# ZJULiHongxin/HRNet-Hand-Pose-Estimation

Measured on AMD Instinct MI355X. Metric: images/sec fwd+bwd pose_hrnet_w32 256x256 bs=64/GPU, higher is better.
Workload: dtype bf16; 1 GPU; pose_hrnet_w32 256x256 bf16 fwd+HeatmapLoss+bwd+Adam training step, batch 64/GPU, synthetic RHD-shaped crops, random-init weights; global_batch=64, parallelism=dp1

## Files before the change

### hrnet-hand-pose-estimation_amd/build.py

```python
import hashlib
import os
import subprocess
import sys
from concurrent.futures import ThreadPoolExecutor

HERE = os.path.dirname(os.path.abspath(__file__))
REPO = os.path.dirname(HERE)
CSRC = os.path.join(HERE, 'csrc')
OBJ = os.path.join(CSRC, 'build')
LIB = os.path.join(CSRC, 'libhrnet_hip.so')
SOURCES = ['api.hip', 'conv.hip', 'conv_bs.hip', 'conv_fwd.hip', 'conv_dg.hip', 'conv_fwdb.hip', 'conv_fwds.hip', 'conv_ring.hip', 'wgrad.hip', 'bwd_fused.hip', 'bwd_pw.hip', 'gemm_pw.hip', 'head_mix.hip', 'eltwise.hip', 'loss.hip', 'dcn.hip', 'preprocess.hip', 'triangulate.hip', 'volumetric.hip', 'conv3d.hip', 'conv3d_train.hip', 'pointwise.hip', 'view_fusion.hip', 'transformer.hip', 'swin.hip', 'nmf.hip']
HEADERS = [os.path.join(CSRC, 'common.h'), os.path.join(CSRC, 'conv_body.h'), os.path.join(CSRC, 'conv_ring.h'), os.path.join(REPO, 'include', 'hrnet_hip.h')]
HIPCC = os.environ.get('HIPCC', '/opt/rocm/bin/hipcc')
FLAGS = ['--offload-arch=gfx950', '-O3', '-std=c++17', '-fPIC', '-fno-gpu-rdc',
         '-I', os.path.join(REPO, 'include'), '-I', CSRC, '-Wno-unused-result']


EXTRA = {}


def _stamp(src):
    h = hashlib.sha1()
    for p in [src] + HEADERS:
        with open(p, 'rb') as f:
            h.update(f.read())
    h.update(' '.join(FLAGS + EXTRA.get(os.path.basename(src), [])).encode())
    return h.hexdigest()


def _compile(name):
    src = os.path.join(CSRC, name)
    obj = os.path.join(OBJ, name.replace('.hip', '.o'))
    stamp_file = obj + '.stamp'
    stamp = _stamp(src)
# ... 31 lines not shown
```

### hrnet-hand-pose-estimation_amd/csrc/common.h

```cpp
#pragma once
#include <stdlib.h>
#include <hip/hip_runtime.h>
#include <stdint.h>

#include "hrnet_hip.h"

typedef __bf16 bf16_t;
typedef float f32x4 __attribute__((ext_vector_type(4)));
typedef float f32x2 __attribute__((ext_vector_type(2)));
typedef __bf16 bf16x8 __attribute__((ext_vector_type(8)));
typedef __bf16 bf16x4 __attribute__((ext_vector_type(4)));
typedef uint32_t u32x4 __attribute__((ext_vector_type(4)));
typedef uint32_t u32x2 __attribute__((ext_vector_type(2)));
typedef u32x4 V16;

#define LDS_AS __attribute__((address_space(3)))

template <typename T>
struct TT;
template <>
struct TT<float> {
  static constexpr int VEC = 4;
  static constexpr int KSTEP = 16;
  static constexpr int ID = HR_F32;
// ... 234 lines not shown
int hr_launch_wgrad(const HrOp& op, hipStream_t s);
int hr_launch_wgrad_reduce(const HrOp& op, hipStream_t s);
int hr_launch_bn_finalize(const HrOp& op, hipStream_t s);
int hr_launch_sum_terms(const HrOp& op, hipStream_t s);
int hr_launch_grad_term(const HrOp& op, hipStream_t s);
int hr_launch_bn_bwd_reduce(const HrOp& op, hipStream_t s);
int hr_launch_bn_bwd_finalize(const HrOp& op, hipStream_t s);
int hr_launch_bilinear_cat(const HrOp& op, hipStream_t s);
int hr_launch_bilinear_cat_bwd(const HrOp& op, hipStream_t s);
int hr_launch_im2col_stem(const HrOp& op, hipStream_t s);
int hr_launch_nhwc_to_nchw(const HrOp& op, hipStream_t s);
int hr_launch_nchw_to_nhwc(const HrOp& op, hipStream_t s);
int hr_launch_pack_weights(const HrOp& op, hipStream_t s);
int hr_launch_bias_grad(const HrOp& op, hipStream_t s);
int hr_launch_fill(const HrOp& op, hipStream_t s);
int hr_launch_pack_table(const HrOp& op, hipStream_t s);
int hr_launch_wgrad_reduce_table(const HrOp& op, hipStream_t s);
int hr_launch_bwd_fused(const HrOp& op, hipStream_t s);
int hr_launch_bwd_pw(const HrOp& op, hipStream_t s);
int hr_launch_conv_sum(const HrOp& op, hipStream_t s);
int hr_gemm_pw_supported(int dtype, int Cin, int Cout);
int hr_gemm_pw(const void* x, const void* w, const float* bias, void* y, float* sums, long long pixels, int Cin,
               int Cout, hipStream_t s);
int hr_launch_bn_finalize_table(const HrOp& op, hipStream_t s);
int hr_launch_ew_table(const HrOp& op, hipStream_t s);
int hr_launch_head_mix(const HrOp& op, hipStream_t s);
int hr_launch_upsample_t(const HrOp& op, hipStream_t s);
int hr_launch_head_bwd(const HrOp& op, hipStream_t s);
int hr_launch_pool_reduce(const HrOp& op, hipStream_t s);
```

### hrnet-hand-pose-estimation_amd/csrc/conv.hip

```cpp
#include <string.h>

#include "conv_body.h"
#include "conv_ring.h"

HR_DEFINE_CONV_LAUNCH(hr_conv_launch_generic, CONV_GENERIC)

namespace {
inline int conv_xcd_runs() {
  static const int v = hr_knob("HRNET_CONV_XCD", 1);
  return v;
}
inline int conv_mode(const ConvArgs& a, bool in_relu) {
  if (a.bs_y) return CONV_BS;
  if (!a.bias && !a.upz && !a.accumulate && a.stats) return CONV_FWD;
  if (a.bias && !a.upz && !a.accumulate) return CONV_FWDB;
  if (!a.bias && !a.in_scale && !a.in_sums && !in_relu && !a.stats) return CONV_DG;
  return CONV_GENERIC;
}

inline int ring_serves(const ConvArgs& a, int dtype, int ks, int stride, int mode, bool in_relu) {
  if (ks != 3 || stride != 1 || a.upz || a.bias || a.in_dy || a.in_dx || !hr_conv_ring_enabled()) return 0;
  const bool raw = !a.in_scale && !a.in_sums && !in_relu;
  if (mode == CONV_BS || (raw && a.accumulate && !a.stats))
    return hr_conv_ring_supported(dtype, a.N, a.H, a.W, a.Cin, a.Cout, 1) ? 2 : 0;
// ... 83 lines not shown
             "conv2d: input batch sums need gamma/beta, no scale/shift arrays, Cin <= %d", HR_CONV_MAXC);
  HR_REQUIRE(!a.in_sums || !a.bs_y, "conv2d: batch-sum input is for forward launches");
  HR_REQUIRE(!a.bs_y || a.stats, "conv2d: backward statistics need a rows buffer");
  HR_REQUIRE(!a.bs_store_masked || a.bs_y, "conv2d: the masked store belongs to a backward-statistics launch");
  HR_REQUIRE(!a.bs_y || (!a.in_scale && !a.bias && !op.i[HR_CONV_I_IN_RELU]),
             "conv2d: backward statistics are for input-gradient launches (no input affine / ReLU / bias)");
  HR_REQUIRE((a.bs_scale == nullptr) == (a.bs_shift == nullptr), "conv2d: mask scale/shift must come together");
  a.N = N; a.H = H; a.W = W; a.Cin = Cin;
  a.Ho = Ho; a.Wo = Wo; a.Cout = Cout;
  a.in_relu = op.i[HR_CONV_I_IN_RELU]; a.upz = upz; a.accumulate = op.i[HR_CONV_I_ACCUMULATE];
  const int mode = conv_mode(a, op.i[HR_CONV_I_IN_RELU] != 0);
  HR_REQUIRE(!a.in_sums || mode == CONV_FWD || mode == CONV_FWDB,
             "conv2d: batch-sum input needs a forward launch that writes statistics or adds a bias");
  const int route = op.i[HR_CONV_I_ROUTE];
  HR_REQUIRE(route >= 0 && route <= 2, "conv2d: bad route %d", route);
  const int rs = route == 1 ? 0 : ring_serves(a, dtype, ks, op.i[HR_CONV_I_STRIDE], mode, op.i[HR_CONV_I_IN_RELU] != 0);
  HR_REQUIRE(route != 2 || rs, "conv2d: the op was recorded for the LDS-ring kernel, which does not serve it now "
             "(hrnet_conv_ring_enable() changed after the plan was recorded: record the plan again)");
  if (rs) return launch_ring(a, op.i[HR_CONV_I_IN_RELU], s);
  if (ks == 1 && stride == 1 && !upz && !a.accumulate && !a.bs_y && !a.in_scale && !a.in_sums &&
      !op.i[HR_CONV_I_IN_RELU] &&
      (!a.stats || a.stats_atomic) && !a.in_dy && !a.in_dx && hr_gemm_pw_supported(dtype, Cin, Cout))
    return hr_gemm_pw(a.x, a.w, a.bias, a.y, a.stats, (long long)N * H * W, Cin, Cout, s);
  const bool s2d = upz && (mode == CONV_BS || mode == CONV_DG);
  if (upz) {
    HR_REQUIRE(ks == 3, "conv2d: upz needs a 3x3 kernel");
    HR_REQUIRE((Ho + 1) / 2 == H && (Wo + 1) / 2 == W, "conv2d: upz shape mismatch");
    stride = s2d ? 4 : 1;
    if (s2d) { a.upz = 0; a.Hz = H; a.Wz = W; }
    else { a.Hz = Ho; a.Wz = Wo; }
  } else {
    const int pad = ks / 2;
    HR_REQUIRE((H + 2 * pad - ks) / stride + 1 == Ho && (W + 2 * pad - ks) / stride + 1 == Wo,
               "conv2d: output %dx%d does not match input %dx%d ks=%d stride=%d", Ho, Wo, H, W, ks, stride);
    a.Hz = H; a.Wz = W;
  }
  const TileChoice tc = choose_tile(N, Ho, Wo, Cout, ks, op.i[HR_CONV_I_STRIDE], op.p[HR_CONV_P_BS_Y] != nullptr, s2d);
  a.tiles_y = (Ho + tc.th - 1) / tc.th;
  a.tiles_x = (Wo + tc.tw - 1) / tc.tw;
  a.total_tiles = N * a.tiles_y * a.tiles_x;
  a.tpw = tc.tpw;
  a.gx = tc.gx;
  a.gy = (Cout + tc.bn - 1) / tc.bn;
  a.xcd_runs = conv_xcd_runs();
  ConvLaunch l;
  l.a = a; l.tc = tc; l.dtype = dtype; l.N = N; l.ks = ks; l.stride = stride;
// ... 140 lines not shown
  op.p[HR_CONV_P_X] = (void*)x; op.p[HR_CONV_P_WGT] = (void*)w; op.p[HR_CONV_P_Y] = y; op.p[HR_CONV_P_STATS] = stats;
  op.p[HR_CONV_P_BS_Y] = (void*)bs_y; op.p[HR_CONV_P_BS_MASK] = (void*)bs_mask;
  op.p[HR_CONV_P_BS_SCALE] = (void*)bs_scale; op.p[HR_CONV_P_BS_SHIFT] = (void*)bs_shift;
  HR_REQUIRE(bs_y, "conv2d_bwdstats: null bs_y");
  return hr_launch_conv(op, (hipStream_t)stream);
}

extern "C" int hrnet_conv_mode(int bwdstats, int has_bias, int upz, int accumulate, int has_stats, int has_affine,
                               int in_relu) {
  ConvArgs a = {};
  a.bs_y = bwdstats ? (const char*)1 : nullptr;
  a.bias = has_bias ? (const float*)1 : nullptr;
  a.upz = upz; a.accumulate = accumulate;
  a.stats = has_stats ? (float*)1 : nullptr;
  a.in_scale = has_affine ? (const float*)1 : nullptr;
  return conv_mode(a, in_relu != 0);
}

extern "C" int hrnet_conv_kernel_name(int dtype, int N, int Ho, int Wo, int Cin, int Cout, int ks, int stride,
                                      int upz, int mode, char* buf, int buflen) {
  if (ks == 1 && stride == 1 && !upz && hr_gemm_pw_supported(dtype, Cin, Cout) &&
      (mode == CONV_FWD || mode == CONV_FWDB || mode == CONV_DG))
    return snprintf(buf, buflen, "gemm_pw_kernel");
  if (ks == 3 && stride == 1 && !upz && mode == CONV_FWDS && hr_conv_ring_sum_supported(dtype, N, Ho, Wo, Cin, Cout)) {
    char tmp[96];
    hr_conv_ring_name(hr_conv_ring_supported(dtype, N, Ho, Wo, Cin, Cout, 0), 0, tmp, sizeof(tmp));
    const int n = (int)strlen(tmp);
    if (n > 1) tmp[n - 1] = 0;
    return snprintf(buf, buflen, "%s, true>", tmp);
  }
  if (ks == 3 && stride == 1 && !upz && hr_conv_ring_enabled()) {
    const int bsm = mode == CONV_BS ? 1 : 0;
    if ((bsm || mode == CONV_FWD || mode == CONV_GENERIC || mode == CONV_DG) &&
        hr_conv_ring_supported(dtype, N, Ho, Wo, Cin, Cout, bsm))
      return hr_conv_ring_name(hr_conv_ring_supported(dtype, N, Ho, Wo, Cin, Cout, bsm), bsm, buf, buflen);
  }
  const bool s2d = upz && (mode == CONV_BS || mode == CONV_DG);
  const TileChoice tc = choose_tile(N, Ho, Wo, Cout, ks, stride, mode == CONV_BS, s2d);
  static const int wp[8] = {4, 2, 2, 2, 2, 0, 4, 2}, wc[8] = {1, 2, 2, 2, 2, 0, 1, 2};
  const int kstride = s2d ? 4 : (ks == 1 || upz) ? 1 : stride;
  const int km = conv_km(dtype, ks, Cin, tc.id);
  static const char* names[6] = {"conv_kernel", "conv_bs_kernel", "conv_fwd_kernel", "conv_dg_kernel", "conv_fwdb_kernel",
                                 "conv_fwds_kernel"};
  return snprintf(buf, buflen, "%s<%s, %d, %d, %d, %d, %d, %d, %d, %d>", names[mode >= 0 && mode < 6 ? mode : 0],
                  dtype == HR_F32 ? "float" : "__bf16", ks, kstride, tc.th, tc.tw, tc.bn, wp[tc.id], wc[tc.id], km);
}
// ... 1 lines not shown
```

### hrnet-hand-pose-estimation_amd/csrc/eltwise.hip

```cpp
#include "common.h"

namespace {

constexpr int EW_BLOCK = 256;
inline unsigned ew_grid(long long n) {
  long long g = (n + EW_BLOCK - 1) / EW_BLOCK;
  if (g > 256LL * 16) g = 256LL * 16;
  if (g < 1) g = 1;
  return (unsigned)g;
}

constexpr int FIN_LANES = 32;
__device__ __forceinline__ void partial_sums(const float* rows, int n, int C, int c, int tl, int cl,
                                             double (*red)[FIN_LANES][32], double& s1, double& s2) {
  double a0 = 0, a1 = 0, b0 = 0, b1 = 0;
  if (c < C) {
    int t = tl;
    for (; t + FIN_LANES < n; t += 2 * FIN_LANES) {
      const float x0 = rows[((size_t)t * 2 + 0) * C + c], y0 = rows[((size_t)t * 2 + 1) * C + c];
      const float x1 = rows[((size_t)(t + FIN_LANES) * 2 + 0) * C + c];
      const float y1 = rows[((size_t)(t + FIN_LANES) * 2 + 1) * C + c];
      a0 += (double)x0; b0 += (double)y0; a1 += (double)x1; b1 += (double)y1;
    }
    if (t < n) {
// ... 918 lines not shown
      const int k = (int)(idx % Cin_pad);
      const int co = (int)(idx / Cin_pad);
      if (co < Cout && k < taps * Cin) {
        const int t = k / Cin, ci = k % Cin;
        val = w[((size_t)co * Cin + ci) * taps + t];
      }
    }
    out[idx] = (T)val;
  }
}

constexpr int PACK_LDS_FLOATS = 4864;
__host__ __device__ inline int pack_nci(int Cout, int taps) {
  for (int p = 16; p > 1; p >>= 1)
    if (Cout * (p * taps + 1) <= PACK_LDS_FLOATS) return p;
  return 1;
}
__host__ __device__ inline int pack_rows(int Cin_pad, int taps) {
  const int r = 2048 / (Cin_pad * taps);
  return r < 1 ? 1 : (r > 8 ? 8 : r);
}

template <typename T>
__global__ __launch_bounds__(256) void pack_table_kernel(const HrPackEnt* tab, int n) {
  __shared__ float buf[PACK_LDS_FLOATS];
  int lo = 0, hi = n - 1;
  while (lo < hi) {
    const int mid = (lo + hi + 1) >> 1;
    if (tab[mid].block0 <= (int)blockIdx.x) lo = mid; else hi = mid - 1;
  }
  const HrPackEnt e = tab[lo];
  const int taps = e.ks * e.ks;
  const float* w = (const float*)e.w;
  T* out = (T*)e.out;
  const int u = (int)blockIdx.x - e.block0;
  if (e.mode == 0) {
    const int nr = pack_rows(e.Cin_pad, taps), co0 = u * nr, rowlen = e.Cin * taps, olen = taps * e.Cin_pad;
    const int rows = e.Cout_pad - co0 < nr ? e.Cout_pad - co0 : nr;
    for (int i = threadIdx.x; i < rows * rowlen; i += 256) {
      const int r = i / rowlen;
      buf[i] = co0 + r < e.Cout ? w[e.ld ? (size_t)(co0 + r) * e.ld + (i - r * rowlen) : (size_t)co0 * rowlen + i] : 0.f;
    }
    __syncthreads();
    T* o = out + (size_t)co0 * olen;
    for (int idx = threadIdx.x; idx < rows * olen; idx += 256) {
      const int r = idx / olen, q = idx - r * olen;
      const int t = q / e.Cin_pad, ci = q - t * e.Cin_pad;
      o[idx] = (T)((co0 + r < e.Cout && ci < e.Cin) ? buf[r * rowlen + ci * taps + t] : 0.f);
    }
  } else if (e.mode == 1) {
    const int per = pack_nci(e.Cout_pad, taps);
    const int ci0 = u * per, span = per * taps, pitch = span + 1;
    const int nci = e.Cin_pad - ci0 < per ? e.Cin_pad - ci0 : per;
    for (int i = threadIdx.x; i < e.Cout * span; i += 256) {
      const int co = i / span, r = i - co * span;
      const int ci = ci0 + r / taps;
      buf[co * pitch + r] = ci < e.Cin ? w[((size_t)co * e.Cin + ci0) * taps + r] : 0.f;
    }
    __syncthreads();
    for (int idx = threadIdx.x; idx < nci * taps * e.Cout_pad; idx += 256) {
      const int co = idx % e.Cout_pad;
      const int tf = (idx / e.Cout_pad) % taps;
      const int cl = idx / (e.Cout_pad * taps);
      out[((size_t)(ci0 + cl) * taps + tf) * e.Cout_pad + co] =
          (T)(co < e.Cout ? buf[co * pitch + cl * taps + (taps - 1 - tf)] : 0.f);
    }
  } else {
    const long long total = (long long)e.Cout_pad * e.Cin_pad;
    const long long base = (long long)u * 1024;
#pragma unroll
    for (int r = 0; r < 4; ++r) {
      const long long idx = base + r * 256 + threadIdx.x;
      if (idx >= total) break;
      const int k = (int)(idx % e.Cin_pad);
      const int co = (int)(idx / e.Cin_pad);
      float val = 0.f;
      if (co < e.Cout && k < taps * e.Cin) val = w[((size_t)co * e.Cin + (k % e.Cin)) * taps + k / e.Cin];
      out[idx] = (T)val;
    }
  }
}

template <typename T>
__global__ __launch_bounds__(256) void colsum_kernel(const char* dy, float* partial, long long pixels,
                                                     int Cp) {
  constexpr int VEC = TT<T>::VEC;
  __shared__ float red[256 * VEC];
  const int cv = Cp / VEC;
  const int rows = 256 / cv;
  const int v = threadIdx.x % cv, row = threadIdx.x / cv;
  float s1[VEC];
#pragma unroll
  for (int j = 0; j < VEC; ++j) s1[j] = 0.f;
  if (row < rows)
    for (long long p = (long long)blockIdx.x * rows + row; p < pixels; p += (long long)gridDim.x * rows) {
      float f[VEC];
      v16_unpack<T>(*(const V16*)(dy + ((size_t)p * Cp + v * VEC) * sizeof(T)), f);
#pragma unroll
      for (int j = 0; j < VEC; ++j) s1[j] += f[j];
    }
#pragma unroll
  for (int j = 0; j < VEC; ++j) red[threadIdx.x * VEC + j] = s1[j];
  __syncthreads();
// ... 264 lines not shown
    if (op.i[HR_GRAD_TERM_I_DTYPE] == HR_F32)
      hipLaunchKernelGGL(grad_term_rows_kernel<float>, dim3(ew_grid(tot2)), dim3(256), 0, s, a);
    else
      hipLaunchKernelGGL(grad_term_rows_kernel<bf16_t>, dim3(ew_grid(tot2)), dim3(256), 0, s, a);
    return hr_check_launch("grad_term");
  }
  if (op.i[HR_GRAD_TERM_I_DTYPE] == HR_F32)
    hipLaunchKernelGGL(grad_term_kernel<float>, dim3(ew_grid(total)), dim3(256), 0, s, a);
  else
    hipLaunchKernelGGL(grad_term_kernel<bf16_t>, dim3(ew_grid(total)), dim3(256), 0, s, a);
  return hr_check_launch("grad_term");
}

extern "C" int hrnet_pack_blocks(int Cout_pad, int Cin_pad, int ks, int mode) {
  if (mode == 0) {
    const int nr = pack_rows(Cin_pad, ks * ks);
    return (Cout_pad + nr - 1) / nr;
  }
  if (mode == 1) {
    const int per = pack_nci(Cout_pad, ks * ks);
    return (Cin_pad + per - 1) / per;
  }
  return (int)(((long long)Cout_pad * Cin_pad + 1023) / 1024);
}

extern "C" int hrnet_reduce_blocks(int N, int H, int W, int C) {
  const long long npix = (long long)N * H * W;
  long long b = npix / 64;
  if (b < 1) b = 1;
  if (b > 2048) b = 2048;
  (void)C;
  return (int)b;
}

int hr_launch_bn_bwd_reduce(const HrOp& op, hipStream_t s) {
  GradArgs a;
  if (int e = fill_grad_args(op, a, true)) return e;
  const int vec = op.i[HR_BN_BWD_REDUCE_I_DTYPE] == HR_F32 ? 4 : 8;
  HR_REQUIRE(a.C / vec <= 256, "bn_bwd_reduce: C=%d too wide", a.C);
  const int blocks = hrnet_reduce_blocks(a.N, a.H, a.W, a.C);
  if (op.i[HR_BN_BWD_REDUCE_I_DTYPE] == HR_F32)
    hipLaunchKernelGGL(bn_bwd_reduce_kernel<float>, dim3(blocks), dim3(256), 0, s, a);
  else
    hipLaunchKernelGGL(bn_bwd_reduce_kernel<bf16_t>, dim3(blocks), dim3(256), 0, s, a);
  return hr_check_launch("bn_bwd_reduce");
}
// ... 395 lines not shown
```

### hrnet-hand-pose-estimation_amd/lib/hipnet/net.py

```python
import torch
import torch.nn as nn

from . import _capi as C
from . import ops
from .engine import BNRec, ConvRec, Plan, Program


class HipNet(object):
    def __init__(self, module, stage_cfg, compute_dtype):
        self.module = module
        self.stage_cfg = stage_cfg
        self.compute_dtype = compute_dtype
        self.dtid = C.dtype_id(compute_dtype)
        C.lib()
        params = list(module.parameters())
        if not params or not params[0].is_cuda:
            raise RuntimeError('pose_hrnet: parameters must live on a HIP device (model.cuda()); '
                               'there is no CPU path')
        self.device = params[0].device
        self.plans = {}
        self.fwd_packed = self.bwd_packed = False
        self._flatten(params)
        self._records()

# ... 50 lines not shown
        self.convs, self.bns, self.bn_list, self.bias_pad = {}, {}, {}, {}
        self.bn_list = []
        skip = tuple(getattr(self.module, 'hip_skip_prefixes', ()))
        for name, m in self.module.named_modules():
            if skip and name.startswith(skip):
                continue
            if isinstance(m, nn.Conv2d):
                r = ConvRec(name, m, stem=(name == 'conv1'))
                es = torch.empty((), dtype=self.compute_dtype).element_size()
                taps = r.ks * r.ks
                nf = r.Cout_pad * (1 if r.stem else taps) * r.Cin_pad
                r.wf = torch.empty(nf * es, dtype=torch.uint8, device=self.device)
                if not r.stem:
                    r.wd = torch.empty(r.Cin_pad * taps * r.Cout_pad * es, dtype=torch.uint8, device=self.device)
                self.convs[name] = r
                if m.bias is not None:
                    self.bias_pad[name] = torch.zeros(r.Cout_pad, dtype=torch.float32, device=self.device)
            elif isinstance(m, nn.BatchNorm2d):
                b = BNRec(name, m, self.device)
                self.bns[name] = b
                self.bn_list.append(b)
        self.pack_f = self._pack_program([(r, 2 if r.stem else 0, r.wf) for r in self.convs.values()])
        self.pack_d = self._pack_program([(r, 1, r.wd) for r in self.convs.values() if r.wd is not None])

    def _pack_program(self, items):
        import ctypes
        ents = (C.HrPackEnt * len(items))()
        block = 0
        for e, item in zip(ents, items):
            r, mode, out = item[:3]
            taps = r.ks * r.ks
            if (mode == 1 and r.Cout_pad * (taps + 1) > 4864) or (mode == 0 and r.Cin * taps > 4864):
                raise ValueError('{}: {} output channels at {}x{} exceed the LDS staging of the weight packer'.format(
                    r.prefix, r.Cout, r.ks, r.ks))
            e.w, e.out = C.ptr(r.mod.weight), C.ptr(out)
            e.Cout, e.Cin, e.ks, e.Cout_pad, e.Cin_pad, e.mode = r.Cout, r.Cin, r.ks, r.Cout_pad, r.Cin_pad, mode
            if len(item) > 3:
                c0, c = item[3], item[4]
                assert r.ks == 1 and mode == 0
                e.w = r.mod.weight.data_ptr() + 4 * c0
                e.Cin, e.Cin_pad, e.ld = c, c, r.Cin
            e.block0 = block
            block += C.call('hrnet_pack_blocks', e.Cout_pad, e.Cin_pad, r.ks, mode)
        raw = bytes(ctypes.string_at(ctypes.addressof(ents), ctypes.sizeof(ents)))
        table = torch.frombuffer(bytearray(raw), dtype=torch.uint8).to(self.device)
        self._tables = getattr(self, '_tables', []) + [table]
        prog = Program()
        prog.add(ops.make(C.OP_PACK_TABLE, dtype=self.dtid, n=len(items), blocks=block, table=C.ptr(table)))
        return prog.finalize()

    def head_slices(self, crec, widths):
        key = (crec.prefix, tuple(widths))
        if getattr(self, '_head_key', None) != key:
            es = torch.empty((), dtype=self.compute_dtype).element_size()
            items, off = [], 0
            self._head_wf = []
            for c in widths:
                out = torch.empty(crec.Cout_pad * c * es, dtype=torch.uint8, device=self.device)
                self._head_wf.append(out)
                items.append((crec, 0, out, off, c))
                off += c
            self._head_pack = self._pack_program(items)
            self._head_key = key
            self._head_pack.run()
        return self._head_wf

    def pack_weights(self, for_backward):
        if not self.fwd_packed:
            self.pack_f.run()
            if getattr(self, '_head_pack', None) is not None:
                self._head_pack.run()
            for name, buf in self.bias_pad.items():
                b = self.convs[name].mod.bias
                buf[:b.numel()].copy_(b.detach())
            self.fwd_packed = True
        if for_backward and not self.bwd_packed:
            self.pack_d.run()
            self.bwd_packed = True

    def mark_weights_dirty(self):
        self.fwd_packed = self.bwd_packed = False

    MAX_PLANS_IN_FLIGHT = 4

    def plan(self, N, H, W, training, need_grad):
        key = (N, H, W, bool(training), bool(need_grad))
        pool = self.plans.setdefault(key, [])
        for p in pool:
            if not (need_grad and p.busy):
                return p
        if len(pool) >= self.MAX_PLANS_IN_FLIGHT:
            raise RuntimeError('pose_hrnet: {} training forwards of shape {} are waiting for their backward; run '
                               'backward (or drop the outputs) before more forwards'.format(len(pool), (N, H, W)))
        p = Plan(self, N, H, W, training, need_grad)
        pool.append(p)
        return p

    def forward(self, x, training, need_grad):
        if x.dim() != 4 or x.shape[1] != 3:
            raise ValueError('pose_hrnet expects (B,3,H,W) input, got {}'.format(tuple(x.shape)))
# ... 38 lines not shown
```

### include/hrnet_hip.h

```cpp
#ifndef HRNET_HIP_H
#define HRNET_HIP_H

#include <stdint.h>

#ifdef __cplusplus
extern "C" {
#endif

#define HR_ABI_VERSION 2
#define HR_HOST

typedef void* hr_stream_t;
typedef int hr_value_t;

enum { HR_F32 = 0, HR_BF16 = 1 };

enum {
  HR_OK = 0,
  HR_E_BADARG = -1,
  HR_E_LAUNCH = -2,
  HR_E_BADOP = -3
};

enum {
// ... 161 lines not shown
void* hrnet_event_create(void);
int hrnet_event_destroy(void* event);

int hrnet_conv2d(int dtype, const void* x, const void* w, const float* in_scale,
                 const float* in_shift, const float* bias, void* y, float* stats, int N, int H,
                 int W, int Cin, int Ho, int Wo, int Cout, int ks, int stride, int upz,
                 int in_relu, int accumulate, hr_stream_t stream);

int hrnet_lincomb_f32(float* out, long long n, int k, HR_HOST const float* const* srcs, HR_HOST const float* coefs,
                      hr_stream_t stream);

int hrnet_conv2d_dilated3x3(int dtype, const void* x, const void* w_taps, long long tap_stride_bytes, void* y,
                            int N, int H, int W, int Cin, int Cout, int dilation, hr_stream_t stream);

int hrnet_conv2d_bwdstats(int dtype, const void* x, const void* w, void* y, float* stats,
                          const void* bs_y, const void* bs_mask, const float* bs_scale,
                          const float* bs_shift, int N, int H, int W, int Cin, int Ho, int Wo,
                          int Cout, int ks, int stride, int upz, int accumulate, hr_stream_t stream);
hr_value_t hrnet_conv_ring_enable(int on);
hr_value_t hrnet_conv_ring_supported(int dtype, int N, int H, int W, int Cin, int Cout);
hr_value_t hrnet_conv_rows_bwdstats(int dtype, int N, int Ho, int Wo, int Cin, int Cout, int ks, int stride);
hr_value_t hrnet_conv_route(int dtype, int N, int Ho, int Wo, int Cin, int Cout, int ks, int stride);
hr_value_t hrnet_conv_ring_sum_enable(int on);

hr_value_t hrnet_conv_kernel_name(int dtype, int N, int Ho, int Wo, int Cin, int Cout, int ks, int stride, int upz,
                                  int mode, HR_HOST char* buf, int buflen);
hr_value_t hrnet_conv_mode(int bwdstats, int has_bias, int upz, int accumulate, int has_stats, int has_affine,
                           int in_relu);
hr_value_t hrnet_wgrad_kernel_name(int dtype, int Ho, int Wo, int Cout, int Cin, int ks, int stride,
                                   HR_HOST char* buf, int buflen);
hr_value_t hrnet_conv_tiles(int N, int Ho, int Wo, int Cout, int ks, int stride);
hr_value_t hrnet_conv_tile_walk(int N, int Ho, int Wo, int Cout, int ks, int stride, int bwdstats, int s2d,
                                HR_HOST int* out5);
hr_value_t hrnet_conv_tiles_bwdstats(int N, int Ho, int Wo, int Cout, int ks, int stride);

int hrnet_conv2d_wgrad(int dtype, const void* x, const void* dy, const float* in_scale,
                       const float* in_shift, float* slabs, int N, int H, int W, int Cin, int Ho,
                       int Wo, int Cout, int ks, int stride, int in_relu, int nsplit,
                       hr_stream_t stream);
hr_value_t hrnet_wgrad_splits(int dtype, int N, int Ho, int Wo, int Cout, int Cin, int ks, int stride);
hr_value_t hrnet_wgrad_tiles(int dtype, int N, int Ho, int Wo, int Cout, int Cin, int ks, int stride);
hr_value_t hrnet_wgrad_blocks_per_split(int dtype, int Ho, int Wo, int Cout, int Cin, int ks, int stride);
int hrnet_wgrad_reduce(const float* slabs, float* grad_oihw, int nsplit, int Cout, int Cin,
                       int ks, int Cout_real, int Cin_real, int kflat, int accumulate,
                       hr_stream_t stream);

// ... 25 lines not shown
                            const void* addend, int mask_out, float* rows, const void* bs_y, float* slabs,
                            long long pixels, int Cin, int Cout, hr_stream_t stream);
int hrnet_conv1x1_bwd_fused_bnref(int dtype, const void* dz, const void* y, const float* coef, const HrBnBwdRef* ref,
                                  const void* x, const float* in_scale, const float* in_shift, int in_relu,
                                  const void* wT, void* dx, const void* addend, int mask_out, float* rows,
                                  const void* bs_y, float* slabs, long long pixels, int Cin, int Cout,
                                  hr_stream_t stream);
hr_value_t hrnet_bwd_pw_supported(int dtype, int Cin, int Cout);
hr_value_t hrnet_bwd_pw_rows_supported(int dtype, int Cin, int Cout);
hr_value_t hrnet_bwd_pw_splits(int dtype, long long pixels, int Cin, int Cout);
hr_value_t hrnet_bwd_pw_kernel_name(int dtype, int Cin, int Cout, HR_HOST char* buf, int buflen);

int hrnet_pack_weights(int dtype, const float* w_oihw, void* packed, int Cout, int Cin, int ks,
                       int Cout_pad, int Cin_pad, int mode, hr_stream_t stream);
typedef struct HrPackEnt {
  const void* w;
  void* out;
  int32_t Cout, Cin, ks, Cout_pad, Cin_pad, mode, block0;
  int32_t ld;
} HrPackEnt;
int hrnet_pack_weights_table(int dtype, const HrPackEnt* table, int n, int total_blocks,
                             hr_stream_t stream);
hr_value_t hrnet_pack_blocks(int Cout_pad, int Cin_pad, int ks, int mode);

typedef struct HrWredEnt {
  const float* slabs;
  float* grad;
  int32_t nsplit, Cout_pad, Cin_pad, ks, Cout, Cin, kflat, accumulate, block0;
  int32_t ld;
} HrWredEnt;
int hrnet_wgrad_reduce_table(const HrWredEnt* table, int n, int total_blocks, hr_stream_t stream);

int hrnet_bn_finalize(const float* stats, int tiles, int C, float count, const float* gamma,
                      const float* beta, float* running_mean, float* running_var,
                      int64_t* num_batches_tracked, float momentum, float eps, int training,
                      float* scale, float* shift, float* save_mean, float* save_invstd,
                      hr_stream_t stream);

int hrnet_conv2d_bnref(int dtype, const void* x, const void* w, const float* in_sums, const float* in_gamma,
                       const float* in_beta, float in_inv_count, float in_eps, const float* bias, void* y,
                       float* out_sums, int N, int H, int W, int Cin, int Ho, int Wo, int Cout, int ks, int stride,
                       int in_relu, hr_stream_t stream);
int hrnet_conv2d_sum(int dtype, const void* x, const void* x2, const void* w, const float* in_scale,
                     const float* in_shift, const float* in_sums, const float* in_gamma, const float* in_beta,
                     float in_inv_count, float in_eps, void* side, void* y, float* stats, int stats_atomic, int N,
                     int H, int W, int Cin, int Cout, int ks, hr_stream_t stream);
// ... 285 lines not shown
```

Measured before the change: 4342 images/sec.

## Add narrow pointwise conv kernel and fused forward/dgrad weight-pack pass

Adds a dedicated MFMA kernel for 1x1 bias convolutions with 16 or 32 output channels (e.g. the heatmap head). It keeps the weights in LDS, applies the input BN affine and ReLU on the fly, and prefetches activations several jobs deep. Separately, it adds a paired weight-pack kernel that reads each fp32 weight tile once into LDS and writes both the forward and the flipped dgrad packed layouts, plus the head slices, replacing two separate pack launches per step. These target a poorly served narrow GEMM and redundant weight reads, at the cost of more code paths to keep consistent.

After: 4385 images/sec (median of 6 runs). Within noise of the previous version (+1.0%).

```diff
diff --git a/hrnet-hand-pose-estimation_amd/build.py b/hrnet-hand-pose-estimation_amd/build.py
--- a/hrnet-hand-pose-estimation_amd/build.py
+++ b/hrnet-hand-pose-estimation_amd/build.py
@@ -9,7 +9,7 @@
 CSRC = os.path.join(HERE, 'csrc')
 OBJ = os.path.join(CSRC, 'build')
 LIB = os.path.join(CSRC, 'libhrnet_hip.so')
-SOURCES = ['api.hip', 'conv.hip', 'conv_bs.hip', 'conv_fwd.hip', 'conv_dg.hip', 'conv_fwdb.hip', 'conv_fwds.hip', 'conv_ring.hip', 'wgrad.hip', 'bwd_fused.hip', 'bwd_pw.hip', 'gemm_pw.hip', 'head_mix.hip', 'eltwise.hip', 'loss.hip', 'dcn.hip', 'preprocess.hip', 'triangulate.hip', 'volumetric.hip', 'conv3d.hip', 'conv3d_train.hip', 'pointwise.hip', 'view_fusion.hip', 'transformer.hip', 'swin.hip', 'nmf.hip']
+SOURCES = ['api.hip', 'conv.hip', 'conv_bs.hip', 'conv_fwd.hip', 'conv_dg.hip', 'conv_fwdb.hip', 'conv_fwds.hip', 'conv_ring.hip', 'wgrad.hip', 'bwd_fused.hip', 'bwd_pw.hip', 'gemm_pw.hip', 'conv_pwn.hip', 'head_mix.hip', 'eltwise.hip', 'loss.hip', 'dcn.hip', 'preprocess.hip', 'triangulate.hip', 'volumetric.hip', 'conv3d.hip', 'conv3d_train.hip', 'pointwise.hip', 'view_fusion.hip', 'transformer.hip', 'swin.hip', 'nmf.hip']
 HEADERS = [os.path.join(CSRC, 'common.h'), os.path.join(CSRC, 'conv_body.h'), os.path.join(CSRC, 'conv_ring.h'), os.path.join(REPO, 'include', 'hrnet_hip.h')]
 HIPCC = os.environ.get('HIPCC', '/opt/rocm/bin/hipcc')
 FLAGS = ['--offload-arch=gfx950', '-O3', '-std=c++17', '-fPIC', '-fno-gpu-rdc',
diff --git a/hrnet-hand-pose-estimation_amd/csrc/common.h b/hrnet-hand-pose-estimation_amd/csrc/common.h
--- a/hrnet-hand-pose-estimation_amd/csrc/common.h
+++ b/hrnet-hand-pose-estimation_amd/csrc/common.h
@@ -280,6 +280,12 @@
 int hr_gemm_pw_supported(int dtype, int Cin, int Cout);
 int hr_gemm_pw(const void* x, const void* w, const float* bias, void* y, float* sums, long long pixels, int Cin,
                int Cout, hipStream_t s);
+int hr_conv_pw_narrow_supported(int dtype, int Cin, int Cout);
+int hr_conv_pw_narrow_name(int Cout, char* buf, int buflen);
+int hr_conv_pw_narrow(const void* x, const void* w, const float* bias, void* y, const float* in_scale,
+                      const float* in_shift, const float* in_sums, const float* in_gamma, const float* in_beta,
+                      float in_inv_count, float in_eps, int in_relu, long long pixels, int Cin, int Cout,
+                      hipStream_t s);
 int hr_launch_bn_finalize_table(const HrOp& op, hipStream_t s);
 int hr_launch_ew_table(const HrOp& op, hipStream_t s);
 int hr_launch_head_mix(const HrOp& op, hipStream_t s);
diff --git a/hrnet-hand-pose-estimation_amd/csrc/conv.hip b/hrnet-hand-pose-estimation_amd/csrc/conv.hip
--- a/hrnet-hand-pose-estimation_amd/csrc/conv.hip
+++ b/hrnet-hand-pose-estimation_amd/csrc/conv.hip
@@ -129,6 +129,10 @@
       !op.i[HR_CONV_I_IN_RELU] &&
       (!a.stats || a.stats_atomic) && !a.in_dy && !a.in_dx && hr_gemm_pw_supported(dtype, Cin, Cout))
     return hr_gemm_pw(a.x, a.w, a.bias, a.y, a.stats, (long long)N * H * W, Cin, Cout, s);
+  if (mode == CONV_FWDB && ks == 1 && stride == 1 && Ho == H && Wo == W && !a.stats && !a.in_dy && !a.in_dx &&
+      hr_conv_pw_narrow_supported(dtype, Cin, Cout))
+    return hr_conv_pw_narrow(a.x, a.w, a.bias, a.y, a.in_scale, a.in_shift, a.in_sums, a.in_gamma, a.in_beta,
+                             a.in_inv_count, a.in_eps, a.in_relu, (long long)N * H * W, Cin, Cout, s);
   const bool s2d = upz && (mode == CONV_BS || mode == CONV_DG);
   if (upz) {
     HR_REQUIRE(ks == 3, "conv2d: upz needs a 3x3 kernel");
@@ -315,6 +319,8 @@
   if (ks == 1 && stride == 1 && !upz && hr_gemm_pw_supported(dtype, Cin, Cout) &&
       (mode == CONV_FWD || mode == CONV_FWDB || mode == CONV_DG))
     return snprintf(buf, buflen, "gemm_pw_kernel");
+  if (ks == 1 && stride == 1 && !upz && mode == CONV_FWDB && hr_conv_pw_narrow_supported(dtype, Cin, Cout))
+    return hr_conv_pw_narrow_name(Cout, buf, buflen);
   if (ks == 3 && stride == 1 && !upz && mode == CONV_FWDS && hr_conv_ring_sum_supported(dtype, N, Ho, Wo, Cin, Cout)) {
     char tmp[96];
     hr_conv_ring_name(hr_conv_ring_supported(dtype, N, Ho, Wo, Cin, Cout, 0), 0, tmp, sizeof(tmp));
diff --git a/hrnet-hand-pose-estimation_amd/csrc/conv_pwn.hip b/hrnet-hand-pose-estimation_amd/csrc/conv_pwn.hip
--- /dev/null
+++ b/hrnet-hand-pose-estimation_amd/csrc/conv_pwn.hip
@@ -0,0 +1,196 @@
+#include <stdio.h>
+
+#include "common.h"
+
+namespace {
+
+struct PwnArgs {
+  const char* x;
+  const char* w;
+  const float* bias;
+  char* y;
+  const float* in_scale;
+  const float* in_shift;
+  const float* in_sums;
+  const float* in_gamma;
+  const float* in_beta;
+  float in_inv_count, in_eps;
+  long long P;
+  int Cin, in_relu;
+};
+
+constexpr int PWN_MAXC = 768;
+constexpr int PWN_PF = 2;
+constexpr int PWN_D = 5;
+constexpr int PWN_JOB = 16 * PWN_PF;
+
+template <int FC>
+__global__ __launch_bounds__(256) void conv_pw_narrow_kernel(PwnArgs a) {
+  extern __shared__ __attribute__((aligned(16))) char lds[];
+  constexpr int LANE_C = 4 * FC;
+  const int tid = threadIdx.x, lane = tid & 63, wave = tid >> 6;
+  const int li = lane & 15, lg = lane >> 4;
+  const int Cin = a.Cin, nk = (Cin + 31) >> 5, kp = nk * 32, rowb = kp * 2 + 16;
+  char* wl = lds;
+  float* tab = (float*)(lds + 16 * FC * rowb);
+
+  const long long njobs = (a.P + PWN_JOB - 1) / PWN_JOB;
+  const long long gstride = (long long)gridDim.x * 4;
+  long long lj = (long long)blockIdx.x * 4 + wave, cj = lj;
+  int lk = 0, ck = 0;
+  V16 buf[PWN_D][PWN_PF];
+  auto issue = [&](V16* b) {
+#pragma unroll
+    for (int pf = 0; pf < PWN_PF; ++pf) {
+      long long p = lj * PWN_JOB + pf * 16 + li;
+      if (p >= a.P) p = a.P - 1;
+      const int c = min(lk * 32 + lg * 8, Cin - 8);
+      b[pf] = *(const V16*)(a.x + ((size_t)p * Cin + c) * 2);
+    }
+    if (++lk == nk) { lk = 0; lj += gstride; }
+  };
+#pragma unroll
+  for (int d = 0; d < PWN_D; ++d) issue(buf[d]);
+
+  const int vpr = kp >> 3;
+  for (int i = tid; i < 16 * FC * vpr; i += 256) {
+    const int q = i / vpr, v = i - q * vpr, r = q & 15, fc = q >> 4;
+    const int co = (r >> 2) * LANE_C + fc * 4 + (r & 3);
+    *(V16*)(wl + q * rowb + v * 16) = v * 8 < Cin ? *(const V16*)(a.w + ((size_t)co * Cin + v * 8) * 2) : v16_zero();
+  }
+  const bool has_affine = a.in_sums != nullptr || a.in_scale != nullptr;
+  for (int c = tid; c < kp; c += 256) {
+    float sc = 1.f, sh = 0.f;
+    if (c >= Cin) {
+      sc = 0.f;
+    } else if (a.in_sums) {
+      float m_, r_, v_;
+      hr_bn_from_sums(a.in_sums, Cin, c, a.in_inv_count, a.in_eps, a.in_gamma[c], a.in_beta[c], sc, sh, m_, r_, v_);
+    } else if (a.in_scale) {
+      sc = a.in_scale[c];
+      sh = a.in_shift[c];
+    }
+    tab[c] = sc;
+    tab[kp + c] = sh;
+  }
+  float bias[LANE_C];
+#pragma unroll
+  for (int k = 0; k < LANE_C; ++k) bias[k] = a.bias[lg * LANE_C + k];
+  __syncthreads();
+
+  const bool in_relu = a.in_relu != 0;
+  f32x4 acc[FC][PWN_PF];
+#pragma unroll
+  for (int fc = 0; fc < FC; ++fc)
+#pragma unroll
+    for (int pf = 0; pf < PWN_PF; ++pf) acc[fc][pf] = f32x4{0.f, 0.f, 0.f, 0.f};
+
+  while (cj < njobs) {
+#pragma unroll
+    for (int d = 0; d < PWN_D; ++d) {
+      if (cj < njobs) {
+        const int c0 = ck * 32 + lg * 8;
+        V16 bf[PWN_PF];
+        if (has_affine || in_relu) {
+          float sc[8], sh[8];
+          *(f32x4*)(sc) = *(const f32x4*)(tab + c0);
+          *(f32x4*)(sc + 4) = *(const f32x4*)(tab + c0 + 4);
+          *(f32x4*)(sh) = *(const f32x4*)(tab + kp + c0);
+          *(f32x4*)(sh + 4) = *(const f32x4*)(tab + kp + c0 + 4);
+#pragma unroll
+          for (int pf = 0; pf < PWN_PF; ++pf) {
+            float f[8];
+            v16_unpack<bf16_t>(buf[d][pf], f);
+#pragma unroll
+            for (int j = 0; j < 8; ++j) {
+              if (has_affine) f[j] = fmaf(f[j], sc[j], sh[j]);
+              if (in_relu) f[j] = f[j] > 0.f ? f[j] : 0.f;
+            }
+            bf[pf] = v16_pack<bf16_t>(f);
+          }
+        } else {
+#pragma unroll
+          for (int pf = 0; pf < PWN_PF; ++pf) bf[pf] = buf[d][pf];
+        }
+        if (c0 >= Cin) {
+#pragma unroll
+          for (int pf = 0; pf < PWN_PF; ++pf) bf[pf] = v16_zero();
+        }
+#pragma unroll
+        for (int fc = 0; fc < FC; ++fc) {
+          const V16 af = *(const V16*)(wl + (fc * 16 + li) * rowb + ck * 64 + lg * 16);
+#pragma unroll
+          for (int pf = 0; pf < PWN_PF; ++pf) acc[fc][pf] = mma16<bf16_t>(af, bf[pf], acc[fc][pf]);
+        }
+        issue(buf[d]);
+        if (++ck == nk) {
+#pragma unroll
+          for (int pf = 0; pf < PWN_PF; ++pf) {
+            const long long p = cj * PWN_JOB + pf * 16 + li;
+            float vals[LANE_C];
+#pragma unroll
+            for (int fc = 0; fc < FC; ++fc) {
+              vals[fc * 4 + 0] = acc[fc][pf].x + bias[fc * 4 + 0];
+              vals[fc * 4 + 1] = acc[fc][pf].y + bias[fc * 4 + 1];
+              vals[fc * 4 + 2] = acc[fc][pf].z + bias[fc * 4 + 2];
+              vals[fc * 4 + 3] = acc[fc][pf].w + bias[fc * 4 + 3];
+              acc[fc][pf] = f32x4{0.f, 0.f, 0.f, 0.f};
+            }
+            if (p < a.P) {
+              char* dst = a.y + ((size_t)p * (16 * FC) + lg * LANE_C) * 2;
+              if constexpr (FC == 2) {
+                *(V16*)dst = v16_pack<bf16_t>(vals);
+              } else {
+                const bf16x4 o = {(bf16_t)vals[0], (bf16_t)vals[1], (bf16_t)vals[2], (bf16_t)vals[3]};
+                *(bf16x4*)dst = o;
+              }
+            }
+          }
+          ck = 0;
+          cj += gstride;
+        }
+      }
+    }
+  }
+}
+
+int g_pwn_enabled = 1;
+
+}
+
+extern "C" int hrnet_conv_pw_narrow_enable(int on) {
+  const int prev = g_pwn_enabled;
+  if (on >= 0) g_pwn_enabled = on ? 1 : 0;
+  return prev;
+}
+
+int hr_conv_pw_narrow_supported(int dtype, int Cin, int Cout) {
+  return g_pwn_enabled && dtype == HR_BF16 && (Cout == 16 || Cout == 32) && Cin % 8 == 0 && Cin >= 64 &&
+         Cin <= PWN_MAXC;
+}
+
+int hr_conv_pw_narrow_name(int Cout, char* buf, int buflen) {
+  return snprintf(buf, buflen, "conv_pw_narrow_kernel<%d>", Cout / 16);
+}
+
+int hr_conv_pw_narrow(const void* x, const void* w, const float* bias, void* y, const float* in_scale,
+                      const float* in_shift, const float* in_sums, const float* in_gamma, const float* in_beta,
+                      float in_inv_count, float in_eps, int in_relu, long long pixels, int Cin, int Cout,
+                      hipStream_t s) {
+  HR_REQUIRE(x && w && y && bias && pixels > 0, "conv_pw_narrow: null pointer / empty shape");
+  HR_REQUIRE(hr_conv_pw_narrow_supported(HR_BF16, Cin, Cout), "conv_pw_narrow: Cin=%d Cout=%d not served", Cin, Cout);
+  PwnArgs a;
+  a.x = (const char*)x; a.w = (const char*)w; a.bias = bias; a.y = (char*)y;
+  a.in_scale = in_scale; a.in_shift = in_shift; a.in_sums = in_sums; a.in_gamma = in_gamma; a.in_beta = in_beta;
+  a.in_inv_count = in_inv_count; a.in_eps = in_eps; a.P = pixels; a.Cin = Cin; a.in_relu = in_relu;
+  const int kp = (Cin + 31) / 32 * 32;
+  const size_t ldsb = (size_t)Cout * (kp * 2 + 16) + (size_t)2 * kp * sizeof(float);
+  const long long jobs = (pixels + PWN_JOB - 1) / PWN_JOB;
+  long long blocks = (jobs + 3) / 4;
+  if (blocks > 1024) blocks = 1024;
+  if (Cout == 32)
+    hipLaunchKernelGGL(conv_pw_narrow_kernel<2>, dim3((unsigned)blocks), dim3(256), ldsb, s, a);
+  else
+    hipLaunchKernelGGL(conv_pw_narrow_kernel<1>, dim3((unsigned)blocks), dim3(256), ldsb, s, a);
+  return hr_check_launch("conv_pw_narrow");
+}
diff --git a/hrnet-hand-pose-estimation_amd/csrc/eltwise.hip b/hrnet-hand-pose-estimation_amd/csrc/eltwise.hip
--- a/hrnet-hand-pose-estimation_amd/csrc/eltwise.hip
+++ b/hrnet-hand-pose-estimation_amd/csrc/eltwise.hip
@@ -964,6 +964,25 @@
 }
 
 template <typename T>
+__device__ __forceinline__ void pack_stem_piece(const HrPackEnt& e, int u) {
+  const int taps = e.ks * e.ks;
+  const float* w = (const float*)e.w;
+  T* out = (T*)e.out;
+  const long long total = (long long)e.Cout_pad * e.Cin_pad;
+  const long long base = (long long)u * 1024;
+#pragma unroll
+  for (int r = 0; r < 4; ++r) {
+    const long long idx = base + r * 256 + threadIdx.x;
+    if (idx >= total) break;
+    const int k = (int)(idx % e.Cin_pad);
+    const int co = (int)(idx / e.Cin_pad);
+    float val = 0.f;
+    if (co < e.Cout && k < taps * e.Cin) val = w[((size_t)co * e.Cin + (k % e.Cin)) * taps + k / e.Cin];
+    out[idx] = (T)val;
+  }
+}
+
+template <typename T>
 __global__ __launch_bounds__(256) void pack_table_kernel(const HrPackEnt* tab, int n) {
   __shared__ float buf[PACK_LDS_FLOATS];
   int lo = 0, hi = n - 1;
@@ -1008,19 +1027,152 @@
           (T)(co < e.Cout ? buf[co * pitch + cl * taps + (taps - 1 - tf)] : 0.f);
     }
   } else {
-    const long long total = (long long)e.Cout_pad * e.Cin_pad;
-    const long long base = (long long)u * 1024;
-#pragma unroll
-    for (int r = 0; r < 4; ++r) {
-      const long long idx = base + r * 256 + threadIdx.x;
-      if (idx >= total) break;
-      const int k = (int)(idx % e.Cin_pad);
-      const int co = (int)(idx / e.Cin_pad);
-      float val = 0.f;
-      if (co < e.Cout && k < taps * e.Cin) val = w[((size_t)co * e.Cin + (k % e.Cin)) * taps + k / e.Cin];
-      out[idx] = (T)val;
-    }
-  }
+    pack_stem_piece<T>(e, u);
+  }
+}
+
+constexpr int PAIR_CO = 32;
+constexpr int PAIR_SPAN = 288;
+__host__ __device__ inline int pair_cit(int taps) {
+  for (int p = 64; p > 1; p >>= 1)
+    if (p * taps <= PAIR_SPAN) return p;
+  return 1;
+}
+
+struct Walk2 {
+  int r, j, q, m, n;
+  __device__ __forceinline__ Walk2(int start, int step, int n_) : n(n_) {
+    r = start / n; j = start - r * n;
+    q = step / n;  m = step - q * n;
+  }
+  __device__ __forceinline__ void next() {
+    r += q; j += m;
+    if (j >= n) { j -= n; ++r; }
+  }
+};
+
+template <typename T, int V>
+__device__ __forceinline__ void pair_store(T* dst, const T* v) {
+  if constexpr (V == 1) {
+    dst[0] = v[0];
+  } else {
+    static_assert(V * sizeof(T) == 16, "pair_store: a 16-byte group");
+    V16 pk;
+    __builtin_memcpy(&pk, v, 16);
+    *(V16*)dst = pk;
+  }
+}
+
+template <typename T, int V, int TAPS, bool DGRAD>
+__device__ __forceinline__ void pair_write(T* out, const T* buf, int pitch, int taps_rt, int na, int run, int a0,
+                                           int j0, int ldo) {
+  const int taps = TAPS ? TAPS : taps_rt;
+  const int ng = run / V;
+  for (Walk2 w((int)threadIdx.x, 256, ng); w.r < na * taps; w.next()) {
+    const int a = w.r / taps, t = w.r - a * taps, j = w.j * V;
+    T v[V];
+#pragma unroll
+    for (int k = 0; k < V; ++k)
+      v[k] = DGRAD ? buf[(j + k) * pitch + a * taps + (taps - 1 - t)] : buf[a * pitch + (j + k) * taps + t];
+    pair_store<T, V>(out + ((size_t)(a0 + a) * taps + t) * ldo + j0 + j, v);
+  }
+}
+
+template <typename T, int TAPS>
+__device__ __forceinline__ void pack_pair_tile(const HrPackEnt& f, const HrPackEnt& d, int u, const HrPackEnt* slices,
+                                               int nsl, T* buf) {
+  constexpr int V = 16 / (int)sizeof(T);
+  const int taps = TAPS ? TAPS : f.ks * f.ks;
+  const int cit = pair_cit(taps), pitch = PAIR_SPAN + 4 / (int)sizeof(T);
+  const int nct = (f.Cin_pad + cit - 1) / cit;
+  const int ct = u / nct, co0 = ct * PAIR_CO, ci0 = (u - ct * nct) * cit;
+  const int nco = min(PAIR_CO, f.Cout_pad - co0), nci = min(cit, f.Cin_pad - ci0);
+  const int vco = max(0, min(nco, f.Cout - co0)), vci = max(0, min(nci, f.Cin - ci0));
+  if (vco < nco || vci < nci) {
+    for (int i = threadIdx.x; i < PAIR_CO * pitch; i += 256) buf[i] = (T)0.f;
+    __syncthreads();
+  }
+  const size_t rowp = (size_t)f.Cin * taps;
+  const float* src = (const float*)f.w + ((size_t)co0 * f.Cin + ci0) * taps;
+  const int L = vci * taps;
+  int lead = L;
+  if ((rowp & 3) == 0) lead = min(L, (int)((4 - (((uintptr_t)src >> 2) & 3)) & 3));
+  const int nv = (L - lead) >> 2, ns = L - 4 * nv;
+  if (nv > 0) {
+    constexpr int NLD = PAIR_CO * PAIR_SPAN / 4 / 256;
+    float4 x[NLD];
+    int at[NLD];
+    Walk2 w((int)threadIdx.x, 256, nv);
+#pragma unroll
+    for (int k = 0; k < NLD; ++k) {
+      at[k] = -1;
+      if (w.r < vco) {
+        const int e = lead + 4 * w.j;
+        at[k] = w.r * pitch + e;
+        x[k] = *(const float4*)(src + w.r * rowp + e);
+      }
+      w.next();
+    }
+#pragma unroll
+    for (int k = 0; k < NLD; ++k)
+      if (at[k] >= 0) {
+        T* b = buf + at[k];
+        b[0] = (T)x[k].x; b[1] = (T)x[k].y; b[2] = (T)x[k].z; b[3] = (T)x[k].w;
+      }
+  }
+  if (ns > 0)
+    for (Walk2 w((int)threadIdx.x, 256, ns); w.r < vco; w.next()) {
+      const int e = w.j < lead ? w.j : w.j + 4 * nv;
+      buf[w.r * pitch + e] = (T)src[w.r * rowp + e];
+    }
+  __syncthreads();
+  T* of = (T*)f.out;
+  if ((f.Cin_pad % V) == 0 && (cit % V) == 0 && ((uintptr_t)of & 15) == 0)
+    pair_write<T, V, TAPS, false>(of, buf, pitch, taps, nco, nci, co0, ci0, f.Cin_pad);
+  else
+    pair_write<T, 1, TAPS, false>(of, buf, pitch, taps, nco, nci, co0, ci0, f.Cin_pad);
+  T* od = (T*)d.out;
+  if ((d.Cout_pad % V) == 0 && ((uintptr_t)od & 15) == 0)
+    pair_write<T, V, TAPS, true>(od, buf, pitch, taps, nci, nco, ci0, co0, d.Cout_pad);
+  else
+    pair_write<T, 1, TAPS, true>(od, buf, pitch, taps, nci, nco, ci0, co0, d.Cout_pad);
+  if (TAPS == 1) {
+    for (int s = 0; s < nsl; ++s) {
+      const HrPackEnt e = slices[s];
+      const int c0 = (int)(((const float*)e.w - (const float*)f.w));
+      const int lo = max(c0, ci0), hi = min(c0 + e.Cin, ci0 + nci);
+      if (hi <= lo) continue;
+      T* os = (T*)e.out + (lo - c0);
+      const T* b = buf + (lo - ci0);
+      if (((lo - c0) % V) == 0 && ((hi - lo) % V) == 0 && (e.Cin_pad % V) == 0 && ((uintptr_t)e.out & 15) == 0)
+        pair_write<T, V, 1, false>(os, b, pitch, 1, nco, hi - lo, co0, 0, e.Cin_pad);
+      else
+        pair_write<T, 1, 1, false>(os, b, pitch, 1, nco, hi - lo, co0, 0, e.Cin_pad);
+    }
+  }
+}
+
+template <typename T>
+__global__ __launch_bounds__(256) void pack_pair_kernel(const HrPackEnt* fwd, const HrPackEnt* dgrad,
+                                                        const int* block0, int n, const HrPackEnt* slices, int nsl,
+                                                        int slice_conv) {
+  __shared__ __attribute__((aligned(16))) T buf[PAIR_CO * (PAIR_SPAN + 4 / (int)sizeof(T))];
+  int lo = 0, hi = n - 1;
+  while (lo < hi) {
+    const int mid = (lo + hi + 1) >> 1;
+    if (block0[mid] <= (int)blockIdx.x) lo = mid; else hi = mid - 1;
+  }
+  const HrPackEnt f = fwd[lo];
+  const int u = (int)blockIdx.x - block0[lo];
+  if (f.mode == 2) {
+    pack_stem_piece<T>(f, u);
+    return;
+  }
+  const HrPackEnt d = dgrad[lo];
+  const int ns = lo == slice_conv ? nsl : 0;
+  if (f.ks == 3) pack_pair_tile<T, 9>(f, d, u, slices, 0, buf);
+  else if (f.ks == 1) pack_pair_tile<T, 1>(f, d, u, slices, ns, buf);
+  else pack_pair_tile<T, 0>(f, d, u, slices, 0, buf);
 }
 
 template <typename T>
@@ -1331,6 +1483,37 @@
     return (Cin_pad + per - 1) / per;
   }
   return (int)(((long long)Cout_pad * Cin_pad + 1023) / 1024);
+}
+
+extern "C" int hrnet_pack_pair_blocks(int Cout_pad, int Cin_pad, int ks, int mode) {
+  if (mode == 2) return hrnet_pack_blocks(Cout_pad, Cin_pad, ks, 2);
+  if (ks < 1 || ks * ks > PAIR_SPAN) return 0;
+  const int cit = pair_cit(ks * ks);
+  return ((Cout_pad + PAIR_CO - 1) / PAIR_CO) * ((Cin_pad + cit - 1) / cit);
+}
+
+static int g_pack_pair = 1;
+extern "C" int hrnet_pack_pair_enable(int on) {
+  const int prev = g_pack_pair;
+  if (on >= 0) g_pack_pair = on ? 1 : 0;
+  return prev;
+}
+
+extern "C" int hrnet_pack_weights_pair(int dtype, const HrPackEnt* fwd, const HrPackEnt* dgrad, const int* block0,
+                                       int n, int total_blocks, const HrPackEnt* slices, int nslices, int slice_conv,
+                                       hr_stream_t stream) {
+  HR_REQUIRE(dtype == HR_F32 || dtype == HR_BF16, "pack_weights_pair: dtype %d", dtype);
+  HR_REQUIRE(fwd && dgrad && block0 && n >= 1 && total_blocks >= 1, "pack_weights_pair: args");
+  HR_REQUIRE(nslices >= 0 && (nslices == 0 || (slices && slice_conv >= 0 && slice_conv < n)),
+             "pack_weights_pair: %d slices of convolution %d of %d", nslices, slice_conv, n);
+  hipStream_t s = (hipStream_t)stream;
+  if (dtype == HR_F32)
+    hipLaunchKernelGGL(pack_pair_kernel<float>, dim3(total_blocks), dim3(256), 0, s, fwd, dgrad, block0, n, slices,
+                       nslices, slice_conv);
+  else
+    hipLaunchKernelGGL(pack_pair_kernel<bf16_t>, dim3(total_blocks), dim3(256), 0, s, fwd, dgrad, block0, n, slices,
+                       nslices, slice_conv);
+  return hr_check_launch("pack_weights_pair");
 }
 
 extern "C" int hrnet_reduce_blocks(int N, int H, int W, int C) {
diff --git a/hrnet-hand-pose-estimation_amd/lib/hipnet/net.py b/hrnet-hand-pose-estimation_amd/lib/hipnet/net.py
--- a/hrnet-hand-pose-estimation_amd/lib/hipnet/net.py
+++ b/hrnet-hand-pose-estimation_amd/lib/hipnet/net.py
@@ -96,6 +96,33 @@
                 self.bn_list.append(b)
         self.pack_f = self._pack_program([(r, 2 if r.stem else 0, r.wf) for r in self.convs.values()])
         self.pack_d = self._pack_program([(r, 1, r.wd) for r in self.convs.values() if r.wd is not None])
+        self._pair = self._pair_tables()
+
+    def _pair_tables(self):
+        import ctypes
+        recs = list(self.convs.values())
+        ents = (C.HrPackEnt * len(recs))()
+        starts, block = [], 0
+        for e, r in zip(ents, recs):
+            if not r.stem:
+                e.w, e.out = C.ptr(r.mod.weight), C.ptr(r.wd)
+                e.Cout, e.Cin, e.ks, e.Cout_pad, e.Cin_pad, e.mode = r.Cout, r.Cin, r.ks, r.Cout_pad, r.Cin_pad, 1
+            nb = C.call('hrnet_pack_pair_blocks', r.Cout_pad, r.Cin_pad, r.ks, 2 if r.stem else 0)
+            if nb < 1:
+                return None
+            starts.append(block)
+            block += nb
+        raw = bytes(ctypes.string_at(ctypes.addressof(ents), ctypes.sizeof(ents)))
+        dgrad = torch.frombuffer(bytearray(raw), dtype=torch.uint8).to(self.device)
+        block0 = torch.tensor(starts, dtype=torch.int32).to(self.device)
+        return dgrad, block0, len(recs), block
+
+    def _pack_pair(self):
+        dgrad, block0, n, blocks = self._pair
+        head = getattr(self, '_head_pack', None)
+        C.call('hrnet_pack_weights_pair', self.dtid, C.ptr(self.pack_f.table), C.ptr(dgrad), C.ptr(block0), n, blocks,
+               C.ptr(head.table) if head is not None else None, len(self._head_wf) if head is not None else 0,
+               self._head_conv if head is not None else -1, C.stream_ptr())
 
     def _pack_program(self, items):
         import ctypes
@@ -121,6 +148,7 @@
         self._tables = getattr(self, '_tables', []) + [table]
         prog = Program()
         prog.add(ops.make(C.OP_PACK_TABLE, dtype=self.dtid, n=len(items), blocks=block, table=C.ptr(table)))
+        prog.table = table
         return prog.finalize()
 
     def head_slices(self, crec, widths):
@@ -135,21 +163,28 @@
                 items.append((crec, 0, out, off, c))
                 off += c
             self._head_pack = self._pack_program(items)
+            self._head_conv = list(self.convs).index(crec.prefix)
             self._head_key = key
             self._head_pack.run()
         return self._head_wf
 
     def pack_weights(self, for_backward):
+        pair = (for_backward and not self.fwd_packed and not self.bwd_packed and self._pair is not None
+                and C.call('hrnet_pack_pair_enable', -1) != 0)
+        if pair:
+            self._pack_pair()
         if not self.fwd_packed:
-            self.pack_f.run()
-            if getattr(self, '_head_pack', None) is not None:
-                self._head_pack.run()
+            if not pair:
+                self.pack_f.run()
+                if getattr(self, '_head_pack', None) is not None:
+                    self._head_pack.run()
             for name, buf in self.bias_pad.items():
                 b = self.convs[name].mod.bias
                 buf[:b.numel()].copy_(b.detach())
             self.fwd_packed = True
         if for_backward and not self.bwd_packed:
-            self.pack_d.run()
+            if not pair:
+                self.pack_d.run()
             self.bwd_packed = True
 
     def mark_weights_dirty(self):
diff --git a/include/hrnet_hip.h b/include/hrnet_hip.h
--- a/include/hrnet_hip.h
+++ b/include/hrnet_hip.h
@@ -207,6 +207,7 @@
 hr_value_t hrnet_conv_rows_bwdstats(int dtype, int N, int Ho, int Wo, int Cin, int Cout, int ks, int stride);
 hr_value_t hrnet_conv_route(int dtype, int N, int Ho, int Wo, int Cin, int Cout, int ks, int stride);
 hr_value_t hrnet_conv_ring_sum_enable(int on);
+hr_value_t hrnet_conv_pw_narrow_enable(int on);
 
 hr_value_t hrnet_conv_kernel_name(int dtype, int N, int Ho, int Wo, int Cin, int Cout, int ks, int stride, int upz,
                                   int mode, HR_HOST char* buf, int buflen);
@@ -278,6 +279,11 @@
 int hrnet_pack_weights_table(int dtype, const HrPackEnt* table, int n, int total_blocks,
                              hr_stream_t stream);
 hr_value_t hrnet_pack_blocks(int Cout_pad, int Cin_pad, int ks, int mode);
+int hrnet_pack_weights_pair(int dtype, const HrPackEnt* fwd, const HrPackEnt* dgrad, const int* block0, int n,
+                            int total_blocks, const HrPackEnt* slices, int nslices, int slice_conv,
+                            hr_stream_t stream);
+hr_value_t hrnet_pack_pair_blocks(int Cout_pad, int Cin_pad, int ks, int mode);
+hr_value_t hrnet_pack_pair_enable(int on);
 
 typedef struct HrWredEnt {
   const float* slabs;
```
